# FARIDKH/Multi-agent-RL-for-FJSP

Measured on AMD Instinct MI355X. Metric: env-steps/sec (all agents) at N parallel envs, 1/2/4/8 MI355X, higher is better.
Workload: dtype int32+f64; 1 GPU; fjsp_step_4096envs; envs_per_gpu=4096, global_envs=4096, num_orders=30, policy=random, steps_per_launch=1024, kernel=k_step_ag<lds,predraw>, bench_step=one rollout batch = 256 env-steps of each of the 4096 envs, env_steps_per_bench_step=1048576, parallelism=env-shard x1 (no data-path collective)

## Files before the change

### multi-agent-rl-for-fjsp_amd/_native.py

```python
import ctypes
import importlib
import os
import subprocess
import sysconfig

HERE = os.path.dirname(os.path.abspath(__file__))
REPO = os.path.dirname(HERE)
LIB_PATH = os.environ.get("FJSP_LIB") or os.path.join(HERE, "libfjsp.so")
SRC = os.path.join(HERE, "csrc", "fjsp_hip.hip")
SRCS = [SRC, os.path.join(HERE, "csrc", "fjsp_policy.hip"), os.path.join(HERE, "csrc", "fjsp_group.hip"),
        os.path.join(HERE, "csrc", "fjsp_episode.hip")]
HEADERS = [os.path.join(HERE, "csrc", h) for h in ("fjsp_env.h", "fjsp_select.h", "fjsp_stepdev.h", "fjsp_stamps.h")] + [
    os.path.join(REPO, "include", "fjsp.h")]

FACADE_SRC = os.path.join(HERE, "csrc", "fjsp_facade.c")
FACADE_PATH = os.path.join(HERE, "_facade" + sysconfig.get_config_var("EXT_SUFFIX"))

HIPCC_FLAGS = ["--offload-arch=gfx950", "-O3", "-std=c++17", "-fPIC", "-shared",
               "-ffp-contract=off", "-Wall", "-Wno-unused-function"]


class FjspNativeError(RuntimeError):
    pass


class fjsp_config(ctypes.Structure):
    _fields_ = [(k, ctypes.c_int32) for k in (
        "num_trays", "tray_capacity", "mask_tray_capacity", "storage_capacity", "step_size",
        "max_episode_steps", "agv_speed", "pt_small", "pt_big", "pt_packaging", "packaging_capacity")]


REWARD_FIELDS = ["order_complete_reward", "throughput_bonus", "time_penalty", "pickup_load_reward",
                 "pickup_tray_complete", "pickup_idle_penalty", "agv_delivery_reward", "agv_move_penalty",
                 "agv_packaging_delivery", "agv_invalid_action", "machine_complete_reward", "machine_start_reward",
                 "machine_idle_penalty", "packaging_complete_reward", "packaging_start_reward",
                 "packaging_idle_penalty"]


class fjsp_reward_weights(ctypes.Structure):
    _fields_ = [(k, ctypes.c_double) for k in REWARD_FIELDS]


OUT_FIELDS = ["obs_i32", "obs_i8", "obs_f32", "masks", "rewards", "term", "trunc", "results",
              "orders_completed", "packaged", "sim_time", "status",
              "next_i32", "next_i8", "next_f32", "next_masks", "feats"]


class fjsp_out(ctypes.Structure):
    _fields_ = [(k, ctypes.c_void_p) for k in OUT_FIELDS]


class fjsp_env_view(ctypes.Structure):
    _fields_ = [(k, ctypes.c_int32) for k in (
        "current_step", "num_orders", "next_order", "orders_completed", "total_packaged",
        "agv_row", "agv_col", "agv_carrying", "agv_tray_count")] + [
        ("status", ctypes.c_uint32), ("orders", ctypes.c_uint32 * 64)]


EXPORTS = ["fjsp_abi_version", "fjsp_last_error", "fjsp_default_config", "fjsp_check_config",
           "fjsp_default_reward_weights", "fjsp_set_reward_weights",
           "fjsp_create", "fjsp_destroy", "fjsp_set_stream", "fjsp_set_option", "fjsp_num_envs", "fjsp_state_bytes",
           "fjsp_reset", "fjsp_step", "fjsp_step_many", "fjsp_gae", "fjsp_gae_f64", "fjsp_mt_get", "fjsp_mt_set",
           "fjsp_read_env", "fjsp_sync", "fjsp_last_kernel_ms", "fjsp_pack_a2c", "fjsp_a2c_layout",
           "fjsp_snapshot_bytes", "fjsp_snapshot", "fjsp_restore", "fjsp_last_kernel", "fjsp_a2c_policy",
           "fjsp_a2c_group_keys", "fjsp_a2c_group_verify", "fjsp_a2c_actor_head",
           "fjsp_a2c_relu_bias_grad", "fjsp_a2c_value_head_grad", "fjsp_faults", "fjsp_gae_shared",
           "fjsp_a2c_policy_step", "fjsp_a2c_group_temp_bytes", "fjsp_a2c_group_sort", "fjsp_a2c_group_runs",
           "fjsp_a2c_run_sums_bytes", "fjsp_a2c_run_sums", "fjsp_a2c_critic_fused", "fjsp_a2c_shard_keys", "fjsp_a2c_record_head", "fjsp_a2c_pack_mfma", "fjsp_a2c_slab_stats",
           "fjsp_a2c_wgrad", "fjsp_server_start", "fjsp_server_step", "fjsp_server_step_actions", "fjsp_server_stop",
           "fjsp_episode_temp_bytes", "fjsp_episode_scan", "fjsp_a2c_actor_head_ppo",
           "fjsp_kpi_carry_words", "fjsp_kpi_scan", "fjsp_step_held", "fjsp_actions",
           "fjsp_schedule_carry_words", "fjsp_schedule_temp_bytes", "fjsp_schedule_scan",
           "fjsp_step_sched", "fjsp_packaging_carry_words", "fjsp_packaging_ring_bytes",
           "fjsp_packaging_temp_bytes", "fjsp_packaging_scan"]
POLICY_ACTOR_DPAD, POLICY_CRITIC_DPAD = 16, 48
POLICY_ACTOR_FLOATS = 3 * 256 * 16 // 2 + 256 + 3 * 256 * 256 // 2 + 256 + 8 * 256 + 16
POLICY_CRITIC_FLOATS = 3 * 256 * 48 // 2 + 256 + 3 * 256 * 256 // 2 + 256 + 3 * 128 * 256 // 2 + 128 + 128 + 16
CRITIC_FUSED_PW = 2 * 256 + 2 * 128 + 4
ABI_VERSION = 14

_lib = None


def _stale():
    if not os.path.exists(LIB_PATH):
        return True
    t = os.path.getmtime(LIB_PATH)
    return any(os.path.getmtime(p) > t for p in SRCS + HEADERS)


def build_facade(force=False):
    if not force and os.path.exists(FACADE_PATH) and os.path.getmtime(FACADE_PATH) >= os.path.getmtime(FACADE_SRC):
        return FACADE_PATH
    import numpy
    r = subprocess.run(["gcc", "-O2", "-shared", "-fPIC", "-Wall", "-Wextra", "-Wno-unused-parameter",
# ... 143 lines not shown
```

### multi-agent-rl-for-fjsp_amd/csrc/fjsp_hip.hip

```cpp
#include <hip/hip_runtime.h>
#include <stdint.h>
#include <stdio.h>
#include <stdlib.h>
#include <string.h>
#include <chrono>
#include <string>
#include <type_traits>

#include "fjsp_env.h"
#include "fjsp_select.h"
#include "fjsp_stamps.h"
#include "fjsp_stepdev.h"
#include "../../include/fjsp.h"

using namespace fjsp;

namespace {

FJSP_DIAG(__device__ unsigned long long g_stamps[8];
          __device__ unsigned long long g_pgstamps[4];
          __device__ unsigned long long g_emitstamps[4];
          __device__ unsigned long long g_agstamps[64];)

__device__ __forceinline__ void spin_until(uint32_t* flag, uint32_t v, uint32_t* abort, const uint32_t* cap) {
// ... 285 lines not shown
    if (e >= S.n) return;
    Env E;
    env_load(E, S.words, S.n, e);
    Tables T;
    if constexpr (LDS) {
        T.orders = s_orders + lane;
        T.scode = s_code + lane;
        T.snext = s_next + lane;
        T.scstep = s_cstep + lane;
        T.stride = BLOCK;
        tables_copy_in(S, T, e, E.norders(), E.slot_next());
    } else {
        T = tables_of(S, e);
    }
    FJSP_DIAG(
    for (int i = 0; i < 8; i++) E.st_acc[i] = 0;
    E.st_t0 = __builtin_amdgcn_s_memtime();
    )
    for (int k = 0; k < K; k++) {
        int act[NA];
        synth_actions(seed, gid0 + (uint32_t)e, step0 + (uint32_t)k, mode, E, T, C, act);
        FJSP_STAMP(E, 0);
        step_and_emit<true, FULL>(E, T, C, S, e, act, nullptr, autoreset, out, (uint32_t)k);
    }
    if constexpr (LDS) {
        for (int o = 0; o < E.norders(); o++) S.orders[(size_t)o * S.n + e] = T.orders[o * BLOCK];
        for (int s = 0; s < E.slot_next(); s++) {
            S.scode[(size_t)s * S.n + e] = T.scode[s * BLOCK];
            S.snext[(size_t)s * S.n + e] = T.snext[s * BLOCK];
            S.scstep[(size_t)s * S.n + e] = T.scstep[s * BLOCK];
        }
    }
    env_store(E, S.words, S.n, e);
    FJSP_DIAG(
    if (lane == 0)
        for (int i = 0; i < 8; i++) atomicAdd((unsigned long long*)&g_stamps[i], (unsigned long long)E.st_acc[i]);
    )
}

template <int PART>
struct PartSink {
    StoreSink s;
    __device__ __forceinline__ void i32(int f, int v) { if (PART <= 0) s.i32(f, v); }
    __device__ __forceinline__ void f32(int f, float v) { if (PART <= 0) s.f32(f, v); }
    __device__ __forceinline__ void i8(int f, int v) { if (PART != 0) s.i8(f, v); }
    __device__ __forceinline__ void mask(int f, int v) { if (PART != 0) s.mask(f, v); }
};

template <uint32_t I32M, uint32_t I8M, uint32_t F32M, uint32_t MKM>
struct FieldSink {
    StoreSink s;
    __device__ __forceinline__ void i32(int f, int v) { if ((I32M >> f) & 1u) s.i32(f, v); }
    __device__ __forceinline__ void f32(int f, float v) { if ((F32M >> f) & 1u) s.f32(f, v); }
    __device__ __forceinline__ void i8(int f, int v) { if ((I8M >> f) & 1u) s.i8(f, v); }
    __device__ __forceinline__ void mask(int f, int v) { if ((MKM >> f) & 1u) s.mask(f, v); }
};

constexpr uint32_t SNAP_WORDS = ((1u << NSTATE) - 1u) & ~((1u << 3) | (0xFu << 13) | (1u << 19) | (3u << 24));
constexpr int SNAP_N = 32;
static_assert(__builtin_popcount(SNAP_WORDS) + NA + 1 <= SNAP_N, "snapshot slot");
struct alignas(16) PipeSnap {
    uint4 q[SNAP_N / 4][BLOCK];
};
__device__ __forceinline__ void snap_put(PipeSnap& sp, int lane, const uint32_t* v) {
#pragma unroll
    for (int g = 0; g < SNAP_N / 4; g++) sp.q[g][lane] = make_uint4(v[4 * g], v[4 * g + 1], v[4 * g + 2], v[4 * g + 3]);
}
__device__ __forceinline__ void snap_get(const PipeSnap& sp, int lane, uint32_t* v) {
#pragma unroll
    for (int g = 0; g < SNAP_N / 4; g++) {
        const uint4 x = sp.q[g][lane];
        v[4 * g] = x.x; v[4 * g + 1] = x.y; v[4 * g + 2] = x.z; v[4 * g + 3] = x.w;
    }
}
constexpr int SNAP_RES = __builtin_popcount(SNAP_WORDS), SNAP_GSTAT = SNAP_RES + NA;

__device__ __forceinline__ uint32_t pack_actions(const int* act, int lo) {
    return (uint32_t)act[lo] | ((uint32_t)act[lo + 1] << 8) | ((uint32_t)act[lo + 2] << 16) | ((uint32_t)act[lo + 3] << 24);
}

constexpr int PG_CR = 1;
constexpr int PG_PB = 8;
constexpr int AG_PB = 4;
template <int CR, int PB, bool FINAL_MB = false, bool ASYNC = false>
__device__ __forceinline__ void predraw_wave(const DevState& S, int K, int lane, int e, bool valid, size_t ebase,
                                             uint32_t (*s_mb)[2][BLOCK], uint4 (*s_cp)[3][BLOCK], uint32_t* s_nxt) {
    const uint32_t n = (uint32_t)S.n;
    int ph = 0, nord = 0, pos = 0, g = 0;
    uint32_t src = 0, my = 0x100u;
    OrderDraw d{0, 0, 0, 0, 0u};
    int ls_prev[CR];
    uint32_t sl_prev[CR];
    bool inflight = false;
    uint4 pfa[(PB + 4) / 4], pfc[(PB + 4) / 4];
    int pf_pa = -1;
    static_assert(!ASYNC || CR == 1, "one row in flight per step");
    uint4 cp0 = make_uint4(0u, 0u, 0u, 0u), cp1 = cp0, cp2 = cp0;
    if (valid) {
        const uint32_t pg = S.words[(size_t)PGW * n + e];
        if (pg & 1u) {
            ph = 3;
            my = 0;
            nord = (int)((pg >> 24) & 0x7Fu);
            pos = (int)((pg >> 1) & 0x3FFu);
            g = (int)((pg >> 11) & 0x3FFu);
            src = ((pg >> 21) & 1u) ^ (nord > 0 ? 1u : 0u);
        }
    }
    FJSP_DIAG(
    uint64_t pg_busy = 0, pg_act = 0, pg_busy_act = 0, pg_ph[3] = {0, 0, 0};
    )
    for (int k = 0; k <= K; k++) {
        FJSP_DIAG(
        const uint64_t pt0 = __builtin_amdgcn_s_memtime();
        bool pg_active = false;
        )
        if (valid) {
            const uint32_t si = s_mb[0][k & 1][lane];
            if ((si & 0xFFu) != my) {
                const uint32_t sw = s_mb[1][k & 1][lane];
                my = si & 0xFFu;
                nord = (int)((si >> 8) & 0x7Fu);
                src = sw >> 31;
                pos = (int)(sw & 0x3FFu);
                g = (int)((sw >> 16) & 0x3FFu);
                d = OrderDraw{0, 0, 0, 0, 0u};
                pf_pa = -1;
                ph = nord > 0 ? 1 : 3;
            }
        }
        auto prefetch = [&](const uint32_t* work) __attribute__((always_inline)) {
            pf_pa = pos & ~3;
            mt_load<PB>(work, pf_pa, pfa, pfc);
        };
        auto draw_step = [&]() __attribute__((always_inline)) {
            if (valid && ph == 2) {
                uint32_t* work = S.mt + ((size_t)(src ^ 1u) * n + e) * MT_N;
                uint32_t v[PB];
                int pa, cnt;
                if (ASYNC && pf_pa == (pos & ~3)) {
                    const int pn = pf_pa + PB >= MT_N ? 0 : pf_pa + PB;
                    uint4 pna[(PB + 4) / 4], pnc[(PB + 4) / 4];
                    mt_load<PB>(work, pn, pna, pnc);
                    mt_batch_loaded<PB>(work, pos, g, v, pa, cnt, pfa, pfc);
#pragma unroll
                    for (int q = 0; q < (PB + 4) / 4; q++) { pfa[q] = pna[q]; pfc[q] = pnc[q]; }
                    pf_pa = pn;
                    pos += draw_orders<PB>(v, pos - pa, cnt, nord, d, s_nxt + lane, BLOCK);
                    if (pos == MT_N) { pos = 0; g = 0; }
                    if (d.o >= nord) { ph = 3; pf_pa = -1; }
                } else {
                    mt_batch<PB>(work, pos, g, v, pa, cnt);
                    pos += draw_orders<PB>(v, pos - pa, cnt, nord, d, s_nxt + lane, BLOCK);
                    if (pos == MT_N) { pos = 0; g = 0; }
                    if (d.o >= nord) ph = 3;
                    if (ASYNC) {
                        if (ph == 2) prefetch(work);
                        else pf_pa = -1;
                    }
                }
            }
        };
        FJSP_DIAG(
        const uint64_t pt1 = __builtin_amdgcn_s_memtime();
        )
        const int promote = ph;
        uint64_t need = __ballot(valid && ph == 1);
        FJSP_DIAG(
        pg_active = need != 0 || __ballot(valid && ph == 2) != 0;
        )
        if (ASYNC) {
            draw_step();
            FJSP_DIAG(
            const uint64_t pt2 = __builtin_amdgcn_s_memtime();
            if (pg_active) { pg_ph[0] += pt1 - pt0; pg_ph[1] += pt2 - pt1; }
            )
            if (ASYNC && inflight) {
                const int pb = (k - 1) & 1;
#pragma unroll
                for (int r = 0; r < CR; r++) {
                    const size_t el = ebase + (size_t)ls_prev[r];
                    uint4* rd = reinterpret_cast<uint4*>(S.mt + ((size_t)(sl_prev[r] ^ 1u) * n + el) * MT_N);
                    rd[lane] = cp0;
                    rd[lane + 64] = cp1;
                    if (lane + 128 < MT_N / 4) rd[lane + 128] = cp2;
                }
                (void)pb;
                inflight = false;
            }

#pragma unroll
            for (int r = 0; r < CR; r++)
                if (promote == 4 && ph == 4 && lane == ls_prev[r]) ph = 2;
            if (valid && promote == 4 && ph == 2)
                prefetch(S.mt + ((size_t)(src ^ 1u) * n + e) * MT_N);
            if (need) {
                const int first = __builtin_ctzll(need);
#pragma unroll
                for (int r = 0; r < CR; r++) {
                    ls_prev[r] = need ? __builtin_ctzll(need) : first;
                    need &= need - 1;
                    sl_prev[r] = (uint32_t)__builtin_amdgcn_readlane((int)src, ls_prev[r]);
                    const size_t el = ebase + (size_t)ls_prev[r];
                    const uint4* rs = reinterpret_cast<const uint4*>(S.mt + ((size_t)sl_prev[r] * n + el) * MT_N);
                    cp0 = rs[lane];
                    cp1 = rs[lane + 64];
                    cp2 = rs[min(lane + 128, MT_N / 4 - 1)];
                    if (lane == ls_prev[r] && ph == 1) ph = 4;
                }
                inflight = true;
            }
        } else if (need) {
            const int first = __builtin_ctzll(need);
            int ls[CR];
#pragma unroll
            for (int r = 0; r < CR; r++) {
                ls[r] = need ? __builtin_ctzll(need) : first;
                need &= need - 1;
                const uint32_t sl = (uint32_t)__builtin_amdgcn_readlane((int)src, ls[r]);
                const size_t el = ebase + (size_t)ls[r];
                const uint4* rs = reinterpret_cast<const uint4*>(S.mt + ((size_t)sl * n + el) * MT_N);
#pragma unroll
                for (int i = 0; i < 3; i++)
                    __builtin_amdgcn_global_load_lds(
                        (__attribute__((address_space(1))) void*)(rs + min(lane + 64 * i, MT_N / 4 - 1)),
                        (__attribute__((address_space(3))) void*)&s_cp[r][i][0], 16, 0, 0);
            }
            draw_step();
            __builtin_amdgcn_s_waitcnt(0x0F70);
#pragma unroll
            for (int r = 0; r < CR; r++) {
                const uint32_t sl = (uint32_t)__builtin_amdgcn_readlane((int)src, ls[r]);
                const size_t el = ebase + (size_t)ls[r];
                uint4* rd = reinterpret_cast<uint4*>(S.mt + ((size_t)(sl ^ 1u) * n + el) * MT_N);
                rd[lane] = s_cp[r][0][lane];
                rd[lane + 64] = s_cp[r][1][lane];
                if (lane + 128 < MT_N / 4) rd[lane + 128] = s_cp[r][2][lane];
                if (lane == ls[r]) ph = 2;
            }
        } else {
            draw_step();
        }
        if (valid) {
            const uint32_t wrow = nord > 0 ? (src ^ 1u) : src;
            s_mb[2][(k + 1) & 1][lane] = (ph == 3 ? 1u : 0u) | (my << 1) | ((uint32_t)nord << 9);
            s_mb[3][(k + 1) & 1][lane] = (uint32_t)pos | ((uint32_t)g << 16) | (wrow << 31);
        }
        FJSP_DIAG(
        {
            const uint64_t dt = __builtin_amdgcn_s_memtime() - pt0;
            pg_busy += dt;
            if (pg_active) { pg_act += 1; pg_busy_act += dt; }
            (void)pg_ph;
        }
        )
        __syncthreads();
    }
    if (ASYNC) __builtin_amdgcn_s_waitcnt(0x0F70);
    FJSP_DIAG(
    if (lane == 0) {
        atomicAdd(&g_pgstamps[0], (unsigned long long)pg_busy);
        atomicAdd(&g_pgstamps[1], (unsigned long long)pg_act);
        atomicAdd(&g_pgstamps[2], (unsigned long long)pg_busy_act);
        atomicAdd(&g_pgstamps[3], (unsigned long long)(K + 1));
        if (ASYNC) { atomicAdd(&g_agstamps[52], (unsigned long long)pg_ph[0]); atomicAdd(&g_agstamps[53], (unsigned long long)pg_ph[1]); }
    }
    )
    if (valid) {
        uint32_t pg = 0;
        if (FINAL_MB && (s_mb[0][(K + 1) & 1][lane] & 0xFFu) != my) ph = 0;
        if (ph == 3) {
            const uint32_t wrow = nord > 0 ? (src ^ 1u) : src;
            pg = 1u | ((uint32_t)pos << 1) | ((uint32_t)g << 11) | (wrow << 21) | ((uint32_t)nord << 24);
            for (int o = 0; o < nord; o++) S.nxt[(size_t)o * n + e] = s_nxt[o * BLOCK + lane];
        }
        S.words[(size_t)PGW * n + e] = pg;
    }
}

__device__ constexpr fjsp_out kNoOutDev = {};
struct PipeArgs {
    DevState S;
    Cfg C;
    int K;
    uint64_t seed;
    uint32_t gid0, step0;
    int mode, autoreset;
    fjsp_out out;
};
struct AgArgs {
    DevState S;
    Cfg C;
    int K;
    uint64_t seed;
    uint32_t gid0, step0;
    int autoreset;
    fjsp_out out;
};
static_assert(sizeof(DevState) == 64 && sizeof(Cfg) == 48 && offsetof(AgArgs, C) == 64 && offsetof(AgArgs, K) == 112 &&
                  offsetof(AgArgs, seed) == 120 && offsetof(AgArgs, gid0) == 128 && offsetof(AgArgs, autoreset) == 136 &&
                  offsetof(AgArgs, out) == 144,
              "AgArgs mirrors k_step_ag's kernel arguments (the kernarg segment's layout)");
static_assert(offsetof(PipeArgs, K) == 112 && offsetof(PipeArgs, seed) == 120 && offsetof(PipeArgs, step0) == 132 &&
                  offsetof(PipeArgs, mode) == 136 && offsetof(PipeArgs, autoreset) == 140 && offsetof(PipeArgs, out) == 144,
              "PipeArgs mirrors k_step_pipe's kernel arguments");
template <class A>
__device__ __forceinline__ const A* kargs_flat() {
    const A* p = (const A*)__builtin_amdgcn_kernarg_segment_ptr();
    asm volatile("" : "+s"(p));
    return p;
}
template <class A>
__device__ __forceinline__ Cfg cfg_at(const A* a, const double* lut) {
    Cfg c = a->C;
    c.lut = lut;
    return c;
}
__device__ __forceinline__ fjsp_out out_at(const fjsp_out& o) {
    fjsp_out r = kNoOutDev;
    r.obs_i32 = o.obs_i32; r.obs_i8 = o.obs_i8; r.obs_f32 = o.obs_f32; r.masks = o.masks;
    r.rewards = o.rewards; r.term = o.term; r.trunc = o.trunc; r.status = o.status;
    return r;
}
#define FJSP_KARG __attribute__((address_space(4)))
template <class A>
__device__ __forceinline__ const FJSP_KARG A* kargs() {
    const FJSP_KARG A* p = (const FJSP_KARG A*)__builtin_amdgcn_kernarg_segment_ptr();
    asm volatile("" : "+s"(p));
    return p;
}
__device__ __forceinline__ const FJSP_KARG AgArgs* ag_args() { return kargs<AgArgs>(); }
template <class A>
__device__ __forceinline__ Cfg cfg_at(const FJSP_KARG A* a, const double* lut) {
    Cfg c;
    c.step_size = a->C.step_size; c.max_steps = a->C.max_steps; c.tray_cap = a->C.tray_cap;
    c.mask_tray_cap = a->C.mask_tray_cap; c.storage_cap = a->C.storage_cap; c.pool0 = a->C.pool0;
    c.pkg_cap = a->C.pkg_cap; c.ptk_small = a->C.ptk_small; c.ptk_big = a->C.ptk_big; c.ptk_pack = a->C.ptk_pack;
    c.lut = lut;
    return c;
}
template <class A>
__device__ __forceinline__ DevState state_at(const FJSP_KARG A* a) {
    DevState s;
    s.words = a->S.words; s.orders = a->S.orders; s.scode = a->S.scode; s.snext = a->S.snext;
    s.scstep = a->S.scstep; s.mt = a->S.mt; s.nxt = a->S.nxt; s.n = a->S.n;
    return s;
}
template <class A>
// ... 658 lines not shown
                    }
                    trunc_prev = step >= C.max_steps;
                    E.set_step(step + 1);
                }
            } else if (kvalid && g == 0) {
                s_kpost[2][el] = E.w[2];
            }
            AG_ACC(ag_busy);
            AG_BARRIER();
        }
        if (kvalid) {
            const uint32_t c01 = lanes_or<G>(pack_lane_counts<G>(E, g, 0)), c23 = lanes_or<G>(pack_lane_counts<G>(E, g, 1));
#pragma unroll
            for (int p = 0; p < NP; p++) {
                const size_t s = (size_t)(p * G + g);
                S.words[(7 + L_PKG + s) * n + ek] = E.w[7 + L_PKG + p];
                S.words[(20 + s) * n + ek] = E.w[20 + p];
                S.words[(26 + s) * n + ek] = E.w[26 + p];
            }
            if (g == 0) {
                S.words[n + ek] = E.w[1];
                S.words[(size_t)24 * n + ek] = c01;
                S.words[(size_t)25 * n + ek] = c23;
            }
        }
    } else if (wave == AG_P) {
        const Cfg C = cfg_at(ag_args(), s_lut);
        __builtin_amdgcn_s_setprio(3);
        uint32_t sa[7] = {0u, 0u, 0u, 0u, 0u, 0u, 0u};
        for (int k = 0; k <= K; k++) {
            AG_T0();
            if (k + 1 < K) {
                const int act1 = (int)((s_act[(k + 1) % 3][0][lane] >> 8) & 0xFFu);
                AG_MARK(0);
                const bool fresh = ag_fresh(k, valid, s_p1, s_kpost, lane, C, autoreset);
                AG_SPIN_T0();
                const bool wait_first = __ballot(valid && fresh) != 0;
                if (wait_first) ag_spin(&s_flag1, (uint32_t)(k + 1));
                AG_MARK(1);
                Env Ea;
#pragma unroll
                for (int i = 0; i < NSTATE; i++) Ea.w[i] = 0u;
                AgvPre pre{};
                if (valid) {
                    if (fresh) {
                        uint32_t p1[8];
                        q_get(&s_p1[k & 1][0][lane], 2, p1);
                        const uint4 p2 = s_p2[lane];
                        sa[0] = p1[P1_W6]; sa[1] = p1[P1_W7]; sa[2] = p1[P1_W8];
                        sa[3] = p2.x; sa[4] = p2.y; sa[5] = p2.z; sa[6] = p2.w;
                    }
#pragma unroll
                    for (int i = 0; i < 7; i++) Ea.w[6 + i] = sa[i];
                    pre = agv_pre(Ea, TL, C, act1);
                }
                ag_pin(pre);
                AG_MARK(2);
                if (!wait_first) ag_spin(&s_flag1, (uint32_t)(k + 1));
                ag_spin(&s_uflag, (uint32_t)(k + 1));
                AG_SPIN_ACC();
                AG_MARK(3);
                if (valid) {
                    const uint4 p2 = s_p2[lane];
                    const uint4 pk = s_pk[lane];
                    const uint2 pr = s_pkr[lane];
                    Ea.w[5] = pk.z; Ea.w[7] = pk.w;
                    Ea.w[9] = p2.x; Ea.w[10] = p2.y; Ea.w[11] = p2.z; Ea.w[12] = p2.w;
                    int mv = 0;
                    uint32_t pend = 0;
                    const uint32_t r1 = agv_fin(Ea, TL, pre, &mv, &pend);
                    AG_MARK(4);
#pragma unroll
                    for (int i = 0; i < 7; i++) sa[i] = Ea.w[6 + i];
                    const uint32_t rs[16] = {pk.x >> 24, pk.y, Ea.w[5], Ea.w[6], Ea.w[7], Ea.w[8], Ea.w[9],
                                             Ea.w[10], Ea.w[11], Ea.w[12], pr.x, r1, pr.y | Ea.w[2], 0u, 0u, pend};
                    q_put(&s_res[(k + 1) & 1][0][lane], 4, rs);
                }
                AG_MARK(5);
            }
            AG_ACC(ag_busy);
            AG_BARRIER();
        }
    } else if (wave == AG_PD) {
        predraw_wave<CR, PB, true, true>(S, K, lane, e, valid, (size_t)blk * EPW, s_mb, s_cp, s_nxt);
    } else {
        auto emit_loop = [&](auto role) __attribute__((always_inline)) {
            constexpr int part = decltype(role)::value;
            const FJSP_KARG AgArgs* ea = ag_args();
            const Cfg C = cfg_at(ea, s_lut);
            if (part == 3) __builtin_amdgcn_s_setprio(2);
            const fjsp_out eo = out_at(ea);
            const uint32_t n = (uint32_t)ea->S.n;
            const uint64_t eseed = ea->seed;
            const uint32_t egid = ea->gid0 + (uint32_t)e, estep = ea->step0;
            for (int k = 0; k <= K; k++) {
                AG_T0();
                if (part == 3 && k + 1 < K) {
                    const bool fresh = ag_fresh(k, valid, s_p1, s_kpost, lane, C, autoreset);
                    if (__ballot(valid && fresh) != 0) ag_spin(&s_flag1, (uint32_t)(k + 1));
                    AG_MARK(3);
                    if (valid) {
                        Env Ep;
#pragma unroll
                        for (int i = 0; i < NSTATE; i++) Ep.w[i] = 0u;
                        if (fresh) {
                            uint32_t p1[8];
                            q_get(&s_p1[k & 1][0][lane], 2, p1);
                            Ep.w[0] = p1[P1_W0]; Ep.w[4] = p1[P1_W4]; Ep.w[5] = p1[P1_W5]; Ep.w[7] = p1[P1_W7];
                        } else {
                            uint32_t rs[16];
                            q_get(&s_res[k & 1][0][lane], 2, rs);
                            Ep.w[0] = (s_p1[(k - 1) & 1][0][lane].x & 0x00FFFFFFu) | (rs[RS_NO] << 24);
                            Ep.w[4] = rs[RS_W4]; Ep.w[5] = rs[RS_W5]; Ep.w[7] = rs[RS_W5 + 2];
                        }
                        const int act0 = (int)(s_act[(k + 1) % 3][0][lane] & 0xFFu);
                        const uint32_t r0 = (pickup_execute(Ep, TL, C, act0) & 0xFFu) | ((uint32_t)act0 << 8);
                        AG_MARK(4);
                        s_pk[lane] = make_uint4(Ep.w[0], Ep.w[4], Ep.w[5], Ep.w[7]);
                        s_pkr[lane] = make_uint2(r0, Ep.w[2]);
                        __hip_atomic_store(&s_uflag, (uint32_t)(k + 1), __ATOMIC_RELEASE, __HIP_MEMORY_SCOPE_WORKGROUP);
                    }
                }
                AG_MARK(0);
                if (part == 0 && k + 2 < K) {
                    int act[NA];
                    synth_uniform(eseed, egid, estep + (uint32_t)(k + 2), act);
                    s_act[(k + 2) % 3][0][lane] = pack_actions(act, 0);
                    s_act[(k + 2) % 3][1][lane] = pack_actions(act, 4);
                }
                if (k > 0 && valid) {
                    const uint32_t t = (uint32_t)(k - 1);
                    uint32_t v[SNAP_N];
                    snap_get(snap[(k - 1) & 1], lane, v);
                    if (part == 2 && s_abort) v[SA_ST] |= ST_SPIN_TIMEOUT | ST_DIVERGED;
                    FJSP_DIAG(
                    __builtin_amdgcn_s_waitcnt(0xc07f);
                    )
                    AG_MARK(1);
                    ag_emit<part, BLOCK / EPW>(v, t, n, ue, C, eo);
                }
                AG_MARK(2);
                AG_ACC(ag_busy);
                AG_BARRIER();
            }
        };
        if (wave == AG_E0) emit_loop(std::integral_constant<int, 0>{});
        else if (wave == AG_E1) emit_loop(std::integral_constant<int, 1>{});
        else if (wave == AG_E2) emit_loop(std::integral_constant<int, 2>{});
        else emit_loop(std::integral_constant<int, 3>{});
    }
    __syncthreads();
    const DevState So = state_at(ag_args());
    if (threadIdx.x == 0) report_abort(So, s_abort);
    FJSP_DIAG(
    const uint64_t t_out = __builtin_amdgcn_s_memtime();
    )
    if (valid) {
        const uint32_t no = s_act[0][0][lane], ns = s_act[0][1][lane];
        for (uint32_t o = (uint32_t)wave; o < no; o += AG_WAVES) So.orders[(size_t)o * n + e] = TL.orders[o * BLOCK];
        for (uint32_t q = (uint32_t)wave; q < ns; q += AG_WAVES) {
            So.scode[(size_t)q * n + e] = TL.scode[q * BLOCK];
            So.snext[(size_t)q * n + e] = TL.snext[q * BLOCK];
            So.scstep[(size_t)q * n + e] = TL.scstep[q * BLOCK];
        }
    }
    FJSP_DIAG(
    const int slot = wave == AG_AM ? 0 : wave == AG_E0 ? 1 : wave == AG_K ? 2 : wave == AG_E1 ? 3 : wave == AG_P ? 4
// ... 1035 lines not shown
```

### multi-agent-rl-for-fjsp_amd/csrc/fjsp_stepdev.h

```cpp
#pragma once
#include <hip/hip_runtime.h>
#include <stdint.h>

#include "fjsp_env.h"
#include "fjsp_stamps.h"
#include "../../include/fjsp.h"

namespace fjsp {

constexpr int MT_N = 624;

struct DevState {
    uint32_t* words;
    uint32_t* orders;
    uint16_t* scode;
    uint8_t* snext;
    uint16_t* scstep;
    uint32_t* mt;
    uint32_t* nxt;
    int n;
};
constexpr int AUX_WORDS = 4, AUX_FAULT = 0, AUX_SPIN_CAP = 1, AUX_TEST_STALL = 2;
__device__ __forceinline__ uint32_t* aux_words(const DevState& S) { return S.words + (size_t)NWORDS * S.n; }
__device__ __forceinline__ void stall_for_test(const DevState& S) {
    const uint32_t s = aux_words(S)[AUX_TEST_STALL];
    for (uint32_t i = 0; i < s; i++) __builtin_amdgcn_s_sleep(127);
}

__device__ __forceinline__ void env_load(Env& E, const uint32_t* __restrict__ w, int n, int e) {
#pragma unroll
    for (int i = 0; i < NSTATE; i++) E.w[i] = w[i * n + e];
}
__device__ __forceinline__ void env_store(const Env& E, uint32_t* __restrict__ w, int n, int e) {
#pragma unroll
    for (int i = 0; i < NSTATE; i++) w[i * n + e] = E.w[i];
}
static_assert(NWORDS >= NSTATE, "state buffer rows");

__device__ inline void mt_seed(uint32_t* __restrict__ mt, int e, uint32_t seed) {
    uint4* row = reinterpret_cast<uint4*>(mt + (size_t)e * MT_N);
    uint32_t x = seed;
    for (int q = 0; q < MT_N / 4; q++) {
        uint32_t v[4];
#pragma unroll
        for (int j = 0; j < 4; j++) {
            const int i = 4 * q + j;
            if (i > 0) x = 1812433253u * (x ^ (x >> 30)) + (uint32_t)i;
            v[j] = x;
        }
        row[q] = make_uint4(v[0], v[1], v[2], v[3]);
    }
}

constexpr int MTB = 32;

template <int B>
__device__ __forceinline__ void mt_load(const uint32_t* __restrict__ roww, int pa, uint4 (&va)[(B + 4) / 4],
                                        uint4 (&vc)[(B + 4) / 4]) {
    const uint4* row = reinterpret_cast<const uint4*>(roww);
#pragma unroll
    for (int q = 0; q < (B + 4) / 4; q++) {
        int ia = pa + 4 * q;
        ia = ia >= MT_N ? ia - MT_N : ia;
        int ic = pa + 396 + 4 * q;
        ic = ic >= MT_N ? ic - MT_N : ic;
        ic = ic >= MT_N ? ic - MT_N : ic;
        va[q] = row[ia >> 2];
        vc[q] = row[ic >> 2];
    }
}

template <int B>
__device__ __forceinline__ void mt_batch_loaded(uint32_t* __restrict__ roww, int pos, int& g, uint32_t (&v)[B], int& pa,
                                                int& cnt, const uint4 (&va)[(B + 4) / 4], const uint4 (&vc)[(B + 4) / 4]) {
    uint4* row = reinterpret_cast<uint4*>(roww);
    pa = pos & ~3;
    cnt = (MT_N - pa) < B ? (MT_N - pa) : B;
    uint32_t a[B + 4], c[B + 4];
#pragma unroll
    for (int q = 0; q < (B + 4) / 4; q++) {
        a[4 * q] = va[q].x; a[4 * q + 1] = va[q].y; a[4 * q + 2] = va[q].z; a[4 * q + 3] = va[q].w;
        c[4 * q] = vc[q].x; c[4 * q + 1] = vc[q].y; c[4 * q + 2] = vc[q].z; c[4 * q + 3] = vc[q].w;
    }
    uint32_t w[B];
#pragma unroll
    for (int j = 0; j < B; j++) {
        const uint32_t y = (a[j] & 0x80000000u) | (a[j + 1] & 0x7fffffffu);
        const uint32_t regen = c[j + 1] ^ (y >> 1) ^ ((y & 1u) ? 0x9908b0dfu : 0u);
        const uint32_t stale = (uint32_t)((pa + j - g) >> 31);
        w[j] = (regen & ~stale) | (a[j] & stale);
        uint32_t t = w[j];
        t ^= t >> 11;
        t ^= (t << 7) & 0x9d2c5680u;
        t ^= (t << 15) & 0xefc60000u;
        t ^= t >> 18;
        v[j] = t;
    }
#pragma unroll
    for (int q = 0; q < B / 4; q++)
        if (4 * q < cnt) row[(pa >> 2) + q] = make_uint4(w[4 * q], w[4 * q + 1], w[4 * q + 2], w[4 * q + 3]);
    if (pa + cnt > g) g = pa + cnt;
}

template <int B>
__device__ __forceinline__ void mt_batch(uint32_t* __restrict__ roww, int pos, int& g, uint32_t (&v)[B], int& pa,
                                         int& cnt) {
    uint4 va[(B + 4) / 4], vc[(B + 4) / 4];
    mt_load<B>(roww, pos & ~3, va, vc);
    mt_batch_loaded<B>(roww, pos, g, v, pa, cnt, va, vc);
}

struct OrderDraw {
    int o, k, np, ty;
    uint32_t last;
};

template <int B>
__device__ __forceinline__ int draw_orders(const uint32_t (&v)[B], int skip, int cnt, int num_orders, OrderDraw& d,
                                           uint32_t* orders, int stride) {
    int used = 0;
#pragma unroll
    for (int j = 0; j < B; j++) {
        const bool act = j >= skip && j < cnt && d.o < num_orders;
        const uint32_t x = v[j] & (d.k == 0 ? 15u : 3u);
        const bool acc = act && x <= (d.k == 0 ? 8u : 2u);
        const bool emit = acc && d.k == 2;
        d.np = (acc && d.k == 0) ? 1 + (int)x : d.np;
        d.ty = (acc && d.k == 1) ? 1 + (int)x : d.ty;
        const uint32_t ow = ow_make(d.np, d.ty, 1 + (int)x);
        d.last = emit ? ow : d.last;
        orders[(d.o < num_orders ? d.o : num_orders - 1) * stride] = d.last;
        d.o += emit ? 1 : 0;
        d.k = acc ? (d.k == 2 ? 0 : d.k + 1) : d.k;
        used += act ? 1 : 0;
    }
    return used;
}

constexpr int PGW = NSTATE;
static_assert(NWORDS > PGW, "state buffer rows");
__device__ __forceinline__ uint32_t* mt_row(const DevState& S, uint32_t w3, int e) {
    return S.mt + ((size_t)(w3 >> 31) * S.n + e) * MT_N;
}

__device__ __forceinline__ void env_reset(Env& E, const Tables& T, const Cfg& C, const DevState& S, int e,
                                          int num_orders, bool clear_pg = true) {
    env_clear(E, C);
    E.set_norders(num_orders);
    const uint32_t w3 = (uint32_t)E.mti();
    uint32_t* roww = mt_row(S, w3, e);
    int pos = (int)(w3 & 0x3FF), g = (int)((w3 >> 16) & 0x3FF);
    OrderDraw d{0, 0, 0, 0, 0u};
    while (d.o < num_orders) {
        uint32_t v[MTB];
        int pa, cnt;
        mt_batch<MTB>(roww, pos, g, v, pa, cnt);
        pos += draw_orders<MTB>(v, pos - pa, cnt, num_orders, d, T.orders, T.stride);
        if (pos == MT_N) { pos = 0; g = 0; }
    }
    E.set_mti((int)((uint32_t)pos | ((uint32_t)g << 16) | (w3 & 0x80000000u)));
    if (clear_pg) S.words[(size_t)PGW * S.n + e] = 0u;
}

__device__ __forceinline__ void env_reset_predrawn(Env& E, const Tables& T, const Cfg& C, int num_orders,
                                                   uint32_t w3, const uint32_t* nxt) {
    env_clear(E, C);
    E.set_norders(num_orders);
    for (int o = 0; o < num_orders; o++) T.orders[o * T.stride] = nxt[o * BLOCK];
    E.set_mti((int)w3);
}

__device__ __forceinline__
Env env_reset_cold(Env E, Tables T, Cfg C, DevState S, int e, int num_orders, bool clear_pg = true) {
    env_reset(E, T, C, S, e, num_orders, clear_pg);
    return E;
}

__device__ __forceinline__ Tables tables_of(const DevState& S, int e) {
    Tables T;
    T.orders = S.orders + e;
    T.scode = S.scode + e;
    T.snext = S.snext + e;
    T.scstep = S.scstep + e;
    T.stride = S.n;
    return T;
}

template <class V>
__device__ __forceinline__ void st32(V* base, uint32_t elem, V v) {
    *reinterpret_cast<V*>(reinterpret_cast<char*>(base) + elem * (uint32_t)sizeof(V)) = v;
}
constexpr int NFEAT = 38;
constexpr int8_t FEAT_OF_I32[NI32] = {5, 6, 4, 3, 2, 0, 1, 11, 12, 9, 18, 19, 17, 16, 10, 13, 7, 14, 8, 15};
constexpr int8_t FEAT_OF_I8[NI8] = {20, 22, 23, 25, 26, 28, 29, 31, 32, 34, 35, 37};
constexpr int8_t FEAT_OF_F32[NF32] = {21, 24, 27, 30, 33, 36};

struct StoreSink {
    int32_t* pi32; int8_t* pi8; float* pf32; int8_t* pmk;
    uint32_t t, n, e;
    float* pfeat = nullptr;
    __device__ __forceinline__ void feat(int c, float v) { if (pfeat) st32(pfeat, (t * NFEAT + (uint32_t)c) * n + e, v); }
    __device__ __forceinline__ void i32(int f, int v) {
        if (pi32) st32(pi32, (t * NI32 + (uint32_t)f) * n + e, (int32_t)v);
        feat(FEAT_OF_I32[f], (float)v);
    }
    __device__ __forceinline__ void i8(int f, int v) {
        if (pi8) st32(pi8, (t * NI8 + (uint32_t)f) * n + e, (int8_t)v);
        feat(FEAT_OF_I8[f], (float)(int8_t)v);
    }
    __device__ __forceinline__ void f32(int f, float v) {
        if (pf32) st32(pf32, (t * NF32 + (uint32_t)f) * n + e, v);
        feat(FEAT_OF_F32[f], v);
    }
    __device__ __forceinline__ void mask(int f, int v) { if (pmk) st32(pmk, (t * NMASK + (uint32_t)f) * n + e, (int8_t)v); }
};


__device__ __forceinline__ uint64_t fmix64(uint64_t z) {
    z ^= z >> 30; z *= 0xBF58476D1CE4E5B9ull;
    z ^= z >> 27; z *= 0x94D049BB133111EBull;
// ... 69 lines not shown
```

Measured before the change: 3.909 billion env-steps/s.

## Split predraw lane into staged load/refill/consume pipeline with alternating steps

Moves the Mersenne Twister draw helpers into a host/device header and wraps the async predraw lane state in a PreDrawLane struct with separate load, refill (regenerate words) and consume (draw orders) stages. When EPW is 16, refill and consume run on alternating iterations, and the next group load is issued after the copy-back. The aim is to spread the MT load latency and the draw compute across steps so the predraw wave is less likely to hold up the per-step barrier. The trade-off is that each order batch now takes more steps to complete, and it adds extra timing instrumentation under the diagnostic macro.

```diff
diff --git a/multi-agent-rl-for-fjsp_amd/_native.py b/multi-agent-rl-for-fjsp_amd/_native.py
--- a/multi-agent-rl-for-fjsp_amd/_native.py
+++ b/multi-agent-rl-for-fjsp_amd/_native.py
@@ -10,7 +10,7 @@
 SRC = os.path.join(HERE, "csrc", "fjsp_hip.hip")
 SRCS = [SRC, os.path.join(HERE, "csrc", "fjsp_policy.hip"), os.path.join(HERE, "csrc", "fjsp_group.hip"),
         os.path.join(HERE, "csrc", "fjsp_episode.hip")]
-HEADERS = [os.path.join(HERE, "csrc", h) for h in ("fjsp_env.h", "fjsp_select.h", "fjsp_stepdev.h", "fjsp_stamps.h")] + [
+HEADERS = [os.path.join(HERE, "csrc", h) for h in ("fjsp_env.h", "fjsp_select.h", "fjsp_stepdev.h", "fjsp_predraw.h", "fjsp_stamps.h")] + [
     os.path.join(REPO, "include", "fjsp.h")]
 
 FACADE_SRC = os.path.join(HERE, "csrc", "fjsp_facade.c")
diff --git a/multi-agent-rl-for-fjsp_amd/csrc/fjsp_hip.hip b/multi-agent-rl-for-fjsp_amd/csrc/fjsp_hip.hip
--- a/multi-agent-rl-for-fjsp_amd/csrc/fjsp_hip.hip
+++ b/multi-agent-rl-for-fjsp_amd/csrc/fjsp_hip.hip
@@ -391,18 +391,24 @@
 constexpr int PG_CR = 1;
 constexpr int PG_PB = 8;
 constexpr int AG_PB = 4;
-template <int CR, int PB, bool FINAL_MB = false, bool ASYNC = false>
+template <int CR, int PB, bool FINAL_MB = false, bool ASYNC = false, bool ALT = false>
 __device__ __forceinline__ void predraw_wave(const DevState& S, int K, int lane, int e, bool valid, size_t ebase,
                                              uint32_t (*s_mb)[2][BLOCK], uint4 (*s_cp)[3][BLOCK], uint32_t* s_nxt) {
     const uint32_t n = (uint32_t)S.n;
-    int ph = 0, nord = 0, pos = 0, g = 0;
+    int ph = 0, nord_ = 0, pos_ = 0, g_ = 0;
     uint32_t src = 0, my = 0x100u;
-    OrderDraw d{0, 0, 0, 0, 0u};
+    OrderDraw d_{0, 0, 0, 0, 0u};
+    static_assert(!ASYNC || PB == PD_B, "the sliced lane draws PD_B words per refill");
+    struct NoLane {};
+    std::conditional_t<ASYNC, PreDrawLane, NoLane> L;
+    if constexpr (ASYNC) L.start(0, 0, 0);
+    int& nord = [&]() -> int& { if constexpr (ASYNC) return L.nord; else return nord_; }();
+    int& pos = [&]() -> int& { if constexpr (ASYNC) return L.pos; else return pos_; }();
+    int& g = [&]() -> int& { if constexpr (ASYNC) return L.g; else return g_; }();
+    OrderDraw& d = [&]() -> OrderDraw& { if constexpr (ASYNC) return L.d; else return d_; }();
     int ls_prev[CR];
     uint32_t sl_prev[CR];
     bool inflight = false;
-    uint4 pfa[(PB + 4) / 4], pfc[(PB + 4) / 4];
-    int pf_pa = -1;
     static_assert(!ASYNC || CR == 1, "one row in flight per step");
     uint4 cp0 = make_uint4(0u, 0u, 0u, 0u), cp1 = cp0, cp2 = cp0;
     if (valid) {
@@ -417,7 +423,8 @@
         }
     }
     FJSP_DIAG(
-    uint64_t pg_busy = 0, pg_act = 0, pg_busy_act = 0, pg_ph[3] = {0, 0, 0};
+    uint64_t pg_busy = 0, pg_act = 0, pg_busy_act = 0, pg_ph[6] = {0, 0, 0, 0, 0, 0};
+    uint64_t pg_wall[2] = {0, 0}, pg_walln[2] = {0, 0}, pg_last = 0, pg_exit = 0;
     )
     for (int k = 0; k <= K; k++) {
         FJSP_DIAG(
@@ -429,45 +436,33 @@
             if ((si & 0xFFu) != my) {
                 const uint32_t sw = s_mb[1][k & 1][lane];
                 my = si & 0xFFu;
-                nord = (int)((si >> 8) & 0x7Fu);
-                src = sw >> 31;
-                pos = (int)(sw & 0x3FFu);
-                g = (int)((sw >> 16) & 0x3FFu);
-                d = OrderDraw{0, 0, 0, 0, 0u};
-                pf_pa = -1;
+                if constexpr (ASYNC) {
+                    src = sw >> 31;
+                    L.start((int)((si >> 8) & 0x7Fu), (int)(sw & 0x3FFu), (int)((sw >> 16) & 0x3FFu));
+                } else {
+                    nord = (int)((si >> 8) & 0x7Fu);
+                    src = sw >> 31;
+                    pos = (int)(sw & 0x3FFu);
+                    g = (int)((sw >> 16) & 0x3FFu);
+                    d = OrderDraw{0, 0, 0, 0, 0u};
+                }
                 ph = nord > 0 ? 1 : 3;
             }
         }
-        auto prefetch = [&](const uint32_t* work) __attribute__((always_inline)) {
-            pf_pa = pos & ~3;
-            mt_load<PB>(work, pf_pa, pfa, pfc);
-        };
         auto draw_step = [&]() __attribute__((always_inline)) {
-            if (valid && ph == 2) {
+            if constexpr (ASYNC) {
+                uint32_t* work = S.mt + ((size_t)(src ^ 1u) * n + e) * MT_N;
+                if (pd_refill_step<ALT>(k) && valid && ph == 2 && L.can_refill()) L.refill(work);
+                if (pd_consume_step<ALT>(k) && valid && ph == 2 && L.can_consume())
+                    if (L.consume(s_nxt + lane, BLOCK)) ph = 3;
+            } else if (valid && ph == 2) {
                 uint32_t* work = S.mt + ((size_t)(src ^ 1u) * n + e) * MT_N;
                 uint32_t v[PB];
                 int pa, cnt;
-                if (ASYNC && pf_pa == (pos & ~3)) {
-                    const int pn = pf_pa + PB >= MT_N ? 0 : pf_pa + PB;
-                    uint4 pna[(PB + 4) / 4], pnc[(PB + 4) / 4];
-                    mt_load<PB>(work, pn, pna, pnc);
-                    mt_batch_loaded<PB>(work, pos, g, v, pa, cnt, pfa, pfc);
-#pragma unroll
-                    for (int q = 0; q < (PB + 4) / 4; q++) { pfa[q] = pna[q]; pfc[q] = pnc[q]; }
-                    pf_pa = pn;
-                    pos += draw_orders<PB>(v, pos - pa, cnt, nord, d, s_nxt + lane, BLOCK);
-                    if (pos == MT_N) { pos = 0; g = 0; }
-                    if (d.o >= nord) { ph = 3; pf_pa = -1; }
-                } else {
-                    mt_batch<PB>(work, pos, g, v, pa, cnt);
-                    pos += draw_orders<PB>(v, pos - pa, cnt, nord, d, s_nxt + lane, BLOCK);
-                    if (pos == MT_N) { pos = 0; g = 0; }
-                    if (d.o >= nord) ph = 3;
-                    if (ASYNC) {
-                        if (ph == 2) prefetch(work);
-                        else pf_pa = -1;
-                    }
-                }
+                mt_batch<PB>(work, pos, g, v, pa, cnt);
+                pos += draw_orders<PB>(v, pos - pa, cnt, nord, d, s_nxt + lane, BLOCK);
+                if (pos == MT_N) { pos = 0; g = 0; }
+                if (d.o >= nord) ph = 3;
             }
         };
         FJSP_DIAG(
@@ -497,12 +492,20 @@
                 (void)pb;
                 inflight = false;
             }
+            FJSP_DIAG(
+            const uint64_t pt3 = __builtin_amdgcn_s_memtime();
+            if (pg_active) pg_ph[2] += pt3 - pt2;
+            )
 
 #pragma unroll
             for (int r = 0; r < CR; r++)
                 if (promote == 4 && ph == 4 && lane == ls_prev[r]) ph = 2;
-            if (valid && promote == 4 && ph == 2)
-                prefetch(S.mt + ((size_t)(src ^ 1u) * n + e) * MT_N);
+            if constexpr (ASYNC)
+                if (valid && ph == 2 && L.wants_load()) L.load(S.mt + ((size_t)(src ^ 1u) * n + e) * MT_N);
+            FJSP_DIAG(
+            const uint64_t pt4 = __builtin_amdgcn_s_memtime();
+            if (pg_active) pg_ph[3] += pt4 - pt3;
+            )
             if (need) {
                 const int first = __builtin_ctzll(need);
 #pragma unroll
@@ -519,6 +522,9 @@
                 }
                 inflight = true;
             }
+            FJSP_DIAG(
+            if (pg_active) pg_ph[4] += __builtin_amdgcn_s_memtime() - pt4;
+            )
         } else if (need) {
             const int first = __builtin_ctzll(need);
             int ls[CR];
@@ -550,20 +556,31 @@
         } else {
             draw_step();
         }
+        FJSP_DIAG(
+        const uint64_t pt5 = __builtin_amdgcn_s_memtime();
+        )
         if (valid) {
             const uint32_t wrow = nord > 0 ? (src ^ 1u) : src;
             s_mb[2][(k + 1) & 1][lane] = (ph == 3 ? 1u : 0u) | (my << 1) | ((uint32_t)nord << 9);
             s_mb[3][(k + 1) & 1][lane] = (uint32_t)pos | ((uint32_t)g << 16) | (wrow << 31);
         }
         FJSP_DIAG(
+        const uint64_t pb0 = __builtin_amdgcn_s_memtime();
         {
-            const uint64_t dt = __builtin_amdgcn_s_memtime() - pt0;
+            const uint64_t dt = pb0 - pt0;
             pg_busy += dt;
-            if (pg_active) { pg_act += 1; pg_busy_act += dt; }
-            (void)pg_ph;
+            if (pg_active) { pg_act += 1; pg_busy_act += dt; pg_ph[5] += pb0 - pt5; }
         }
         )
         __syncthreads();
+        FJSP_DIAG(
+        {
+            const uint64_t pb1 = __builtin_amdgcn_s_memtime();
+            pg_last += (pb1 - pb0) < 200 ? 1 : 0;
+            if (k > 0) { pg_wall[pg_active ? 0 : 1] += pb1 - pg_exit; pg_walln[pg_active ? 0 : 1] += 1; }
+            pg_exit = pb1;
+        }
+        )
     }
     if (ASYNC) __builtin_amdgcn_s_waitcnt(0x0F70);
     FJSP_DIAG(
@@ -572,7 +589,15 @@
         atomicAdd(&g_pgstamps[1], (unsigned long long)pg_act);
         atomicAdd(&g_pgstamps[2], (unsigned long long)pg_busy_act);
         atomicAdd(&g_pgstamps[3], (unsigned long long)(K + 1));
-        if (ASYNC) { atomicAdd(&g_agstamps[52], (unsigned long long)pg_ph[0]); atomicAdd(&g_agstamps[53], (unsigned long long)pg_ph[1]); }
+        if (ASYNC) {
+            constexpr int PH_SLOT[6] = {52, 53, 54, 55, 50, 51};
+            for (int i = 0; i < 6; i++) atomicAdd(&g_agstamps[PH_SLOT[i]], (unsigned long long)pg_ph[i]);
+            atomicAdd(&g_agstamps[25 + 5], (unsigned long long)pg_last);
+            for (int i = 0; i < 2; i++) {
+                atomicAdd(&g_agstamps[59 + i], (unsigned long long)pg_wall[i]);
+                atomicAdd(&g_agstamps[61 + i], (unsigned long long)pg_walln[i]);
+            }
+        }
     }
     )
     if (valid) {
@@ -1397,7 +1422,7 @@
             AG_BARRIER();
         }
     } else if (wave == AG_PD) {
-        predraw_wave<CR, PB, true, true>(S, K, lane, e, valid, (size_t)blk * EPW, s_mb, s_cp, s_nxt);
+        predraw_wave<CR, PB, true, true, EPW == 16>(S, K, lane, e, valid, (size_t)blk * EPW, s_mb, s_cp, s_nxt);
     } else {
         auto emit_loop = [&](auto role) __attribute__((always_inline)) {
             constexpr int part = decltype(role)::value;
diff --git a/multi-agent-rl-for-fjsp_amd/csrc/fjsp_predraw.h b/multi-agent-rl-for-fjsp_amd/csrc/fjsp_predraw.h
--- /dev/null
+++ b/multi-agent-rl-for-fjsp_amd/csrc/fjsp_predraw.h
@@ -0,0 +1,150 @@
+#pragma once
+#include <stdint.h>
+
+#include "fjsp_env.h"
+
+namespace fjsp {
+
+#ifndef __HIP__
+struct alignas(16) uint4 {
+    uint32_t x, y, z, w;
+};
+inline uint4 make_uint4(uint32_t x, uint32_t y, uint32_t z, uint32_t w) { return uint4{x, y, z, w}; }
+#endif
+
+constexpr int MT_N = 624;
+
+constexpr int MTB = 32;
+
+template <int B>
+FJSP_HD void mt_load(const uint32_t* __restrict__ roww, int pa, uint4 (&va)[(B + 4) / 4], uint4 (&vc)[(B + 4) / 4]) {
+    const uint4* row = reinterpret_cast<const uint4*>(roww);
+#pragma unroll
+    for (int q = 0; q < (B + 4) / 4; q++) {
+        int ia = pa + 4 * q;
+        ia = ia >= MT_N ? ia - MT_N : ia;
+        int ic = pa + 396 + 4 * q;
+        ic = ic >= MT_N ? ic - MT_N : ic;
+        ic = ic >= MT_N ? ic - MT_N : ic;
+        va[q] = row[ia >> 2];
+        vc[q] = row[ic >> 2];
+    }
+}
+
+template <int B>
+FJSP_HD void mt_batch_loaded(uint32_t* __restrict__ roww, int pos, int& g, uint32_t (&v)[B], int& pa, int& cnt,
+                             const uint4 (&va)[(B + 4) / 4], const uint4 (&vc)[(B + 4) / 4]) {
+    uint4* row = reinterpret_cast<uint4*>(roww);
+    pa = pos & ~3;
+    cnt = (MT_N - pa) < B ? (MT_N - pa) : B;
+    uint32_t a[B + 4], c[B + 4];
+#pragma unroll
+    for (int q = 0; q < (B + 4) / 4; q++) {
+        a[4 * q] = va[q].x; a[4 * q + 1] = va[q].y; a[4 * q + 2] = va[q].z; a[4 * q + 3] = va[q].w;
+        c[4 * q] = vc[q].x; c[4 * q + 1] = vc[q].y; c[4 * q + 2] = vc[q].z; c[4 * q + 3] = vc[q].w;
+    }
+    uint32_t w[B];
+#pragma unroll
+    for (int j = 0; j < B; j++) {
+        const uint32_t y = (a[j] & 0x80000000u) | (a[j + 1] & 0x7fffffffu);
+        const uint32_t regen = c[j + 1] ^ (y >> 1) ^ ((y & 1u) ? 0x9908b0dfu : 0u);
+        const uint32_t stale = (uint32_t)((pa + j - g) >> 31);
+        w[j] = (regen & ~stale) | (a[j] & stale);
+        uint32_t t = w[j];
+        t ^= t >> 11;
+        t ^= (t << 7) & 0x9d2c5680u;
+        t ^= (t << 15) & 0xefc60000u;
+        t ^= t >> 18;
+        v[j] = t;
+    }
+#pragma unroll
+    for (int q = 0; q < B / 4; q++)
+        if (4 * q < cnt) row[(pa >> 2) + q] = make_uint4(w[4 * q], w[4 * q + 1], w[4 * q + 2], w[4 * q + 3]);
+    if (pa + cnt > g) g = pa + cnt;
+}
+
+template <int B>
+FJSP_HD void mt_batch(uint32_t* __restrict__ roww, int pos, int& g, uint32_t (&v)[B], int& pa, int& cnt) {
+    uint4 va[(B + 4) / 4], vc[(B + 4) / 4];
+    mt_load<B>(roww, pos & ~3, va, vc);
+    mt_batch_loaded<B>(roww, pos, g, v, pa, cnt, va, vc);
+}
+
+struct OrderDraw {
+    int o, k, np, ty;
+    uint32_t last;
+};
+
+template <int B>
+FJSP_HD int draw_orders(const uint32_t (&v)[B], int skip, int cnt, int num_orders, OrderDraw& d, uint32_t* orders,
+                        int stride) {
+    int used = 0;
+#pragma unroll
+    for (int j = 0; j < B; j++) {
+        const bool act = j >= skip && j < cnt && d.o < num_orders;
+        const uint32_t x = v[j] & (d.k == 0 ? 15u : 3u);
+        const bool acc = act && x <= (d.k == 0 ? 8u : 2u);
+        const bool emit = acc && d.k == 2;
+        d.np = (acc && d.k == 0) ? 1 + (int)x : d.np;
+        d.ty = (acc && d.k == 1) ? 1 + (int)x : d.ty;
+        const uint32_t ow = ow_make(d.np, d.ty, 1 + (int)x);
+        d.last = emit ? ow : d.last;
+        orders[(d.o < num_orders ? d.o : num_orders - 1) * stride] = d.last;
+        d.o += emit ? 1 : 0;
+        d.k = acc ? (d.k == 2 ? 0 : d.k + 1) : d.k;
+        used += act ? 1 : 0;
+    }
+    return used;
+}
+
+constexpr int PD_B = 4;
+struct PreDrawLane {
+    int pos, g, nord;
+    OrderDraw d;
+    int pf_pa;
+    int hcnt;
+    int hpa;
+    uint4 ra[(PD_B + 4) / 4], rc[(PD_B + 4) / 4];
+    uint32_t v[PD_B];
+
+    FJSP_HD void start(int num_orders, int pos0, int g0) {
+        nord = num_orders;
+        pos = pos0;
+        g = g0;
+        d = OrderDraw{0, 0, 0, 0, 0u};
+        pf_pa = -1;
+        hcnt = 0;
+    }
+    FJSP_HD bool done() const { return d.o >= nord; }
+    FJSP_HD int next_group() const { return hcnt != 0 ? (hpa + PD_B >= MT_N ? 0 : hpa + PD_B) : (pos & ~3); }
+    FJSP_HD bool wants_load() const { return hcnt != 0 ? pf_pa == hpa : pf_pa != (pos & ~3); }
+    FJSP_HD bool can_refill() const { return hcnt == 0 && pf_pa == (pos & ~3); }
+    FJSP_HD bool can_consume() const { return hcnt != 0; }
+    FJSP_HD void load(const uint32_t* __restrict__ work) {
+        pf_pa = next_group();
+        mt_load<PD_B>(work, pf_pa, ra, rc);
+    }
+    FJSP_HD void refill(uint32_t* __restrict__ work) {
+#ifdef __HIP_DEVICE_COMPILE__
+        typedef uint32_t u32x4 __attribute__((ext_vector_type(4)));
+        u32x4 t = {rc[0].x, rc[0].y, rc[0].z, rc[0].w};
+        asm volatile("" : "+v"(t));
+        rc[0] = make_uint4(t.x, t.y, t.z, t.w);
+#endif
+        mt_batch_loaded<PD_B>(work, pos, g, v, hpa, hcnt, ra, rc);
+    }
+    FJSP_HD bool consume(uint32_t* orders, int stride) {
+        pos += draw_orders<PD_B>(v, pos - hpa, hcnt, nord, d, orders, stride);
+        if (pos == MT_N) { pos = 0; g = 0; }
+        hcnt = 0;
+        if (done()) pf_pa = -1;
+        return done();
+    }
+};
+
+template <bool ALTERNATE>
+FJSP_HD bool pd_refill_step(int k) { return !ALTERNATE || (k & 1) == 0; }
+template <bool ALTERNATE>
+FJSP_HD bool pd_consume_step(int k) { return !ALTERNATE || (k & 1) != 0; }
+
+}
diff --git a/multi-agent-rl-for-fjsp_amd/csrc/fjsp_stepdev.h b/multi-agent-rl-for-fjsp_amd/csrc/fjsp_stepdev.h
--- a/multi-agent-rl-for-fjsp_amd/csrc/fjsp_stepdev.h
+++ b/multi-agent-rl-for-fjsp_amd/csrc/fjsp_stepdev.h
@@ -3,12 +3,11 @@
 #include <stdint.h>
 
 #include "fjsp_env.h"
+#include "fjsp_predraw.h"
 #include "fjsp_stamps.h"
 #include "../../include/fjsp.h"
 
 namespace fjsp {
-
-constexpr int MT_N = 624;
 
 struct DevState {
     uint32_t* words;
@@ -52,90 +51,6 @@
     }
 }
 
-constexpr int MTB = 32;
-
-template <int B>
-__device__ __forceinline__ void mt_load(const uint32_t* __restrict__ roww, int pa, uint4 (&va)[(B + 4) / 4],
-                                        uint4 (&vc)[(B + 4) / 4]) {
-    const uint4* row = reinterpret_cast<const uint4*>(roww);
-#pragma unroll
-    for (int q = 0; q < (B + 4) / 4; q++) {
-        int ia = pa + 4 * q;
-        ia = ia >= MT_N ? ia - MT_N : ia;
-        int ic = pa + 396 + 4 * q;
-        ic = ic >= MT_N ? ic - MT_N : ic;
-        ic = ic >= MT_N ? ic - MT_N : ic;
-        va[q] = row[ia >> 2];
-        vc[q] = row[ic >> 2];
-    }
-}
-
-template <int B>
-__device__ __forceinline__ void mt_batch_loaded(uint32_t* __restrict__ roww, int pos, int& g, uint32_t (&v)[B], int& pa,
-                                                int& cnt, const uint4 (&va)[(B + 4) / 4], const uint4 (&vc)[(B + 4) / 4]) {
-    uint4* row = reinterpret_cast<uint4*>(roww);
-    pa = pos & ~3;
-    cnt = (MT_N - pa) < B ? (MT_N - pa) : B;
-    uint32_t a[B + 4], c[B + 4];
-#pragma unroll
-    for (int q = 0; q < (B + 4) / 4; q++) {
-        a[4 * q] = va[q].x; a[4 * q + 1] = va[q].y; a[4 * q + 2] = va[q].z; a[4 * q + 3] = va[q].w;
-        c[4 * q] = vc[q].x; c[4 * q + 1] = vc[q].y; c[4 * q + 2] = vc[q].z; c[4 * q + 3] = vc[q].w;
-    }
-    uint32_t w[B];
-#pragma unroll
-    for (int j = 0; j < B; j++) {
-        const uint32_t y = (a[j] & 0x80000000u) | (a[j + 1] & 0x7fffffffu);
-        const uint32_t regen = c[j + 1] ^ (y >> 1) ^ ((y & 1u) ? 0x9908b0dfu : 0u);
-        const uint32_t stale = (uint32_t)((pa + j - g) >> 31);
-        w[j] = (regen & ~stale) | (a[j] & stale);
-        uint32_t t = w[j];
-        t ^= t >> 11;
-        t ^= (t << 7) & 0x9d2c5680u;
-        t ^= (t << 15) & 0xefc60000u;
-        t ^= t >> 18;
-        v[j] = t;
-    }
-#pragma unroll
-    for (int q = 0; q < B / 4; q++)
-        if (4 * q < cnt) row[(pa >> 2) + q] = make_uint4(w[4 * q], w[4 * q + 1], w[4 * q + 2], w[4 * q + 3]);
-    if (pa + cnt > g) g = pa + cnt;
-}
-
-template <int B>
-__device__ __forceinline__ void mt_batch(uint32_t* __restrict__ roww, int pos, int& g, uint32_t (&v)[B], int& pa,
-                                         int& cnt) {
-    uint4 va[(B + 4) / 4], vc[(B + 4) / 4];
-    mt_load<B>(roww, pos & ~3, va, vc);
-    mt_batch_loaded<B>(roww, pos, g, v, pa, cnt, va, vc);
-}
-
-struct OrderDraw {
-    int o, k, np, ty;
-    uint32_t last;
-};
-
-template <int B>
-__device__ __forceinline__ int draw_orders(const uint32_t (&v)[B], int skip, int cnt, int num_orders, OrderDraw& d,
-                                           uint32_t* orders, int stride) {
-    int used = 0;
-#pragma unroll
-    for (int j = 0; j < B; j++) {
-        const bool act = j >= skip && j < cnt && d.o < num_orders;
-        const uint32_t x = v[j] & (d.k == 0 ? 15u : 3u);
-        const bool acc = act && x <= (d.k == 0 ? 8u : 2u);
-        const bool emit = acc && d.k == 2;
-        d.np = (acc && d.k == 0) ? 1 + (int)x : d.np;
-        d.ty = (acc && d.k == 1) ? 1 + (int)x : d.ty;
-        const uint32_t ow = ow_make(d.np, d.ty, 1 + (int)x);
-        d.last = emit ? ow : d.last;
-        orders[(d.o < num_orders ? d.o : num_orders - 1) * stride] = d.last;
-        d.o += emit ? 1 : 0;
-        d.k = acc ? (d.k == 2 ? 0 : d.k + 1) : d.k;
-        used += act ? 1 : 0;
-    }
-    return used;
-}
 
 constexpr int PGW = NSTATE;
 static_assert(NWORDS > PGW, "state buffer rows");
```

Measured after the change: 4.158 billion env-steps/s (median of 6 runs). 6.4% higher.
